# hohMiyazawa/hoh-ANS

Measured on NVIDIA B200. Metric: raw RGB MB/s, encode+decode (BASELINE.json: raw RGB MB/s encode & decode, % of HBM peak), higher is better.
Workload: dtype u8/u16 pixels, u32 freqs, u64 rANS state (integer)

## Files before the change

hoh-ans_b200/build.py:

```python
import os
import shutil
import subprocess
import sys

HERE = os.path.dirname(os.path.abspath(__file__))
CSRC = os.path.join(HERE, "csrc")
LIB = os.path.join(CSRC, "libhohgpu.so")
SOURCES = ["hoh_api.cu"]
DEPS = ["hoh_api.cu", "hoh_kernels.cuh", "hoh_format.cuh", os.path.join("..", "..", "include", "hohgpu.h")]


def nvcc_path():
    for cand in (shutil.which("nvcc"), "/usr/local/cuda/bin/nvcc"):
        if cand and os.path.exists(cand):
            return cand
    raise RuntimeError("nvcc not found")


def stale():
    if not os.path.exists(LIB):
        return True
    t = os.path.getmtime(LIB)
    return any(os.path.getmtime(os.path.join(CSRC, d)) > t for d in DEPS)


def build(force=False, verbose=False):
    if not force and not stale():
        return LIB
    cmd = [nvcc_path(), "-gencode", "arch=compute_100a,code=sm_100a", "-lineinfo", "-O3", "-std=c++17",
           "-Xcompiler", "-fPIC", "-shared", "-cudart", "static", "-o", LIB] + SOURCES
    if verbose:
        cmd.insert(1, "-Xptxas=-v")
    subprocess.check_call(cmd, cwd=CSRC)
    return LIB


if __name__ == "__main__":
    print(build(force="--force" in sys.argv, verbose="-v" in sys.argv))
```

hoh-ans_b200/csrc/hoh_api.cu:

```cuda
#include <cuda_runtime.h>

#include <algorithm>
#include <cmath>
#include <cstdio>
#include <cstdlib>
#include <cstring>
#include <map>
#include <string>
#include <vector>

#include "hoh_kernels.cuh"

using namespace hohk;

namespace {

enum Slot {
    S_FREQS = 0, S_CUM, S_HEADS, S_ENCMETA, S_DECMETA, S_RESID, S_STREAMS, S_DSTREAMS, S_DRESULTS,
    S_IO_A, S_IO_B, S_IO_C, S_IO_D, S_IO_E, S_RESULTS, S_TOP, S_BP, S_HIST, S_COST, S_SUMS, S_MASKS,
    S_WIDE_TOP, S_WIDE_BP, S_MISC, S_L_MAPS, S_L_IDX, S_L_HDR, S_L_U32, S_L_STATUS, S_L_RR, S_L_RES, S_LZ_PX, S_LZ_STATE, S_LZ_SIDE, S_LZ_COUNTS, S_LZ_SLABS, S_LZ_RES, S_LZ_BONUS, S_LZ_KEYS, S_LZ_VALS, S_LZ_FLAG, S_T_NUKE, S_T_LZ, S_T_U32, S_T_P8, S_T_P9, S_T_O8, S_T_O9, S_T_R8, S_T_R9, S_T_MORE_SHAPES, S_T_LAST = S_T_NUKE + 4 * 9 - 1, S_D_TILES, S_D_PLANES, S_D_LZSYM, S_D_IDXSYM, S_D_RESID, S_D_OUT, S_D_BACKREF, S_D_MAPS,
    S_D_STREAMS, S_D_RES_A, S_D_RES_B, S_D_TOP, S_D_BP, S_D_PSTATUS, S_L_NEED, S_L_ORDER, S_R_SLOTS, S_R_STATUS, S_COUNT
};

struct Buf {
// ... 441 lines not shown
namespace {
int predict_all_parallel(hoh_ctx* ctx, const uint16_t* d_planes, size_t n_planes, int w, int h, int depth, int x_tiles,
                         int y_tiles, const uint16_t* d_tile_maps, uint16_t* d_resid, uint64_t resid_stride) {
    const uint64_t tpr = ((uint64_t)w + kPaTx - 1) / kPaTx, tpp = tpr * (((uint64_t)h + kPaTy - 1) / kPaTy);
    if (n_planes * tpp > 0x7fffffffull) return HOH_E_UNSUPPORTED;
    k_predict_all_fused<<<(unsigned)(n_planes * tpp), 256, 0, ctx->stream>>>(
        d_planes, n_planes, w, h, depth, x_tiles, y_tiles, d_tile_maps, d_resid, resid_stride, fastdiv_make((uint32_t)tpp),
        fastdiv_make((uint32_t)tpr), fastdiv_make((uint32_t)((w + x_tiles - 1) / x_tiles)),
        fastdiv_make((uint32_t)((h + y_tiles - 1) / y_tiles)));
    LAUNCHED("k_predict_all_fused");
    return HOH_OK;
}

template <typename T>
int stage_in(hoh_ctx* ctx, Slot slot, const T* host, size_t count, T** dev) {
    TRY(scratch_t(ctx, slot, count ? count : 1, dev));
    if (count) CK(cudaMemcpyAsync(*dev, host, count * sizeof(T), cudaMemcpyHostToDevice, ctx->stream));
    return HOH_OK;
}
template <typename T>
int stage_out(hoh_ctx* ctx, T* host, const T* dev, size_t count) {
    if (count) CK(cudaMemcpyAsync(host, dev, count * sizeof(T), cudaMemcpyDeviceToHost, ctx->stream));
    CK(cudaStreamSynchronize(ctx->stream));
    return HOH_OK;
}
}

namespace {
int new_shape(hoh_ctx* ctx, uint64_t key, uint64_t& slot) {
    if (slot == key) return HOH_OK;
    if (slot != 0) {
        CK(cudaStreamSynchronize(ctx->stream));
        hoh_ctx* who[3] = {ctx, ctx->child[0], ctx->child[1]};
        for (hoh_ctx* c : who) {
            if (!c) continue;
            CK(cudaStreamSynchronize(c->stream));
            for (auto& b : c->scratch) {
                if (b.p) CK(cudaFree(b.p));
                b.p = nullptr;
                b.cap = 0;
            }
        }
    }
    slot = key;
    return HOH_OK;
}

int child_of(hoh_ctx* ctx, int k, hoh_ctx** out) {
    if (!ctx->child[k]) {
        if (hoh_ctx_create(ctx->device, nullptr, &ctx->child[k]) != HOH_OK) return HOH_E_CUDA;
        ctx->child[k]->parent = ctx;
    }
    *out = ctx->child[k];
    return HOH_OK;
}
}

extern "C" {

int hoh_ctx_create(int device, void* cuda_stream, hoh_ctx** out) {
    if (!out) return HOH_E_ARG;
    *out = nullptr;
    int count = 0;
    cudaError_t e = cudaGetDeviceCount(&count);
    if (e != cudaSuccess || count <= 0 || device < 0 || device >= count) return HOH_E_CUDA;
    if (cudaSetDevice(device) != cudaSuccess) return HOH_E_CUDA;
    hoh_ctx* ctx = new hoh_ctx();
    ctx->device = device;
    if (cudaDeviceGetAttribute(&ctx->sm_count, cudaDevAttrMultiProcessorCount, device) != cudaSuccess || ctx->sm_count <= 0)
        ctx->sm_count = 148;
    if (cuda_stream) {
        ctx->stream = reinterpret_cast<cudaStream_t>(cuda_stream);
    } else {
        if (cudaStreamCreateWithFlags(&ctx->stream, cudaStreamNonBlocking) != cudaSuccess) {
            delete ctx;
            return HOH_E_CUDA;
        }
        ctx->own_stream = true;
    }
    *out = ctx;
    return HOH_OK;
}

void hoh_ctx_destroy(hoh_ctx* ctx) {
    if (!ctx) return;
    cudaSetDevice(ctx->device);
    cudaStreamSynchronize(ctx->stream);
    for (auto& b : ctx->scratch)
        if (b.p) cudaFree(b.p);
    for (auto& kv : ctx->e_tabs) cudaFree(kv.second);
    if (ctx->flush) cudaFree(ctx->flush);
    if (ctx->d_layer_stats) cudaFree(ctx->d_layer_stats);
    for (auto& pair : ctx->ev)
        for (auto& ev : pair)
            if (ev) cudaEventDestroy(ev);
    for (auto ev : ctx->prof_events) cudaEventDestroy(ev);
    for (auto ev : ctx->prof_pool) cudaEventDestroy(ev);
    for (hoh_ctx* ch : ctx->child)
        if (ch) hoh_ctx_destroy(ch);
    if (ctx->s_h2d) cudaStreamDestroy(ctx->s_h2d);
    if (ctx->s_d2h) cudaStreamDestroy(ctx->s_d2h);
    for (int k = 0; k < kPipeDepth; k++) {
        if (ctx->ev_h2d[k]) cudaEventDestroy(ctx->ev_h2d[k]);
        if (ctx->ev_comp[k]) cudaEventDestroy(ctx->ev_comp[k]);
        if (ctx->ev_d2h[k]) cudaEventDestroy(ctx->ev_d2h[k]);
        if (ctx->ev_off[k]) cudaEventDestroy(ctx->ev_off[k]);
        if (ctx->h_off[k]) cudaFreeHost(ctx->h_off[k]);
    }
    if (ctx->ev_start) cudaEventDestroy(ctx->ev_start);
    for (int k = 0; k < 8; k++) {
        if (ctx->aux[k]) cudaStreamDestroy(ctx->aux[k]);
        if (ctx->ev_join[k]) cudaEventDestroy(ctx->ev_join[k]);
    }
    if (ctx->ev_fork) cudaEventDestroy(ctx->ev_fork);
    if (ctx->own_stream) cudaStreamDestroy(ctx->stream);
    delete ctx;
}

int hoh_release_scratch(hoh_ctx* ctx) {
    DeviceGuard guard_(ctx);
    if (!ctx) return HOH_E_ARG;
    CK(cudaStreamSynchronize(ctx->stream));
    for (auto& b : ctx->scratch) {
        if (b.p) CK(cudaFree(b.p));
        b.p = nullptr;
        b.cap = 0;
    }
    for (hoh_ctx* ch : ctx->child)
        if (ch) TRY(hoh_release_scratch(ch));
    return HOH_OK;
}

int hoh_sync(hoh_ctx* ctx) {
    DeviceGuard guard_(ctx);
    if (!ctx) return HOH_E_ARG;
    CK(cudaStreamSynchronize(ctx->stream));
    return HOH_OK;
}

const char* hoh_strerror(int status) {
    switch (status) {
        case HOH_OK: return "ok";
        case HOH_E_CUDA: return "CUDA runtime error (no device, or a call failed)";
        case HOH_E_ARG: return "bad argument";
        case HOH_E_UNSUPPORTED: return "outside the supported domain of the hot path";
        case HOH_E_CAPACITY: return "output buffer too small";
        case HOH_E_STREAM: return "a stream failed (see per-stream status)";
        default: return "unknown status";
    }
}

const char* hoh_last_cuda_error(hoh_ctx* ctx) { return ctx ? ctx->err : "no context"; }
uint64_t hoh_launch_count(hoh_ctx* ctx) { return ctx ? ctx->launches : 0; }

int hoh_debug_layer_stats(hoh_ctx* ctx, uint64_t out[3]) {
    if (!ctx || !out) return HOH_E_ARG;
    DeviceGuard guard_(ctx);
    out[0] = out[1] = out[2] = 0;
    hoh_ctx* all[5] = {ctx, ctx->child[0], ctx->child[1], ctx->child[2], ctx->child[3]};
    for (hoh_ctx* c : all) {
        if (!c || !c->d_layer_stats) continue;
        uint32_t v[4];
        CK(cudaStreamSynchronize(c->stream));
        CK(cudaMemcpy(v, c->d_layer_stats, sizeof v, cudaMemcpyDeviceToHost));
        CK(cudaMemset(c->d_layer_stats, 0, sizeof v));
        for (int k = 0; k < 3; k++) out[k] += v[k];
    }
    return HOH_OK;
}

int hoh_dev_alloc(hoh_ctx* ctx, size_t bytes, void** dptr) {
    DeviceGuard guard_(ctx);
    if (!ctx || !dptr) return HOH_E_ARG;
    CK(cudaSetDevice(ctx->device));
    CK(cudaMalloc(dptr, bytes ? bytes : 16));
    return HOH_OK;
}
int hoh_dev_free(hoh_ctx* ctx, void* dptr) {
    DeviceGuard guard_(ctx);
    if (!ctx) return HOH_E_ARG;
    CK(cudaStreamSynchronize(ctx->stream));
    CK(cudaFree(dptr));
    return HOH_OK;
}
int hoh_dev_memset(hoh_ctx* ctx, void* dptr, int value, size_t bytes) {
    DeviceGuard guard_(ctx);
    if (!ctx) return HOH_E_ARG;
    CK(cudaMemsetAsync(dptr, value, bytes, ctx->stream));
    return HOH_OK;
}
int hoh_host_alloc(hoh_ctx* ctx, size_t bytes, void** hptr) {
    DeviceGuard guard_(ctx);
    if (!ctx || !hptr) return HOH_E_ARG;
    CK(cudaHostAlloc(hptr, bytes ? bytes : 16, cudaHostAllocDefault));
    return HOH_OK;
}
int hoh_host_free(hoh_ctx* ctx, void* hptr) {
    DeviceGuard guard_(ctx);
    if (!ctx) return HOH_E_ARG;
    CK(cudaFreeHost(hptr));
    return HOH_OK;
}
int hoh_h2d(hoh_ctx* ctx, void* dst_dev, const void* src_host, size_t bytes) {
    DeviceGuard guard_(ctx);
    if (!ctx) return HOH_E_ARG;
    CK(cudaMemcpyAsync(dst_dev, src_host, bytes, cudaMemcpyHostToDevice, ctx->stream));
    return HOH_OK;
}
int hoh_d2h(hoh_ctx* ctx, void* dst_host, const void* src_dev, size_t bytes) {
    DeviceGuard guard_(ctx);
    if (!ctx) return HOH_E_ARG;
    CK(cudaMemcpyAsync(dst_host, src_dev, bytes, cudaMemcpyDeviceToHost, ctx->stream));
    return HOH_OK;
}
int hoh_timer_start(hoh_ctx* ctx, int slot) {
    DeviceGuard guard_(ctx);
    if (!ctx || slot < 0 || slot >= 16) return HOH_E_ARG;
    for (int k = 0; k < 2; k++)
        if (!ctx->ev[slot][k]) CK(cudaEventCreate(&ctx->ev[slot][k]));
    CK(cudaEventRecord(ctx->ev[slot][0], ctx->stream));
    return HOH_OK;
}
int hoh_timer_stop(hoh_ctx* ctx, int slot) {
    DeviceGuard guard_(ctx);
    if (!ctx || slot < 0 || slot >= 16 || !ctx->ev[slot][1]) return HOH_E_ARG;
    CK(cudaEventRecord(ctx->ev[slot][1], ctx->stream));
    return HOH_OK;
}
int hoh_timer_elapsed_ms(hoh_ctx* ctx, int slot, float* ms) {
    DeviceGuard guard_(ctx);
    if (!ctx || slot < 0 || slot >= 16 || !ms || !ctx->ev[slot][1]) return HOH_E_ARG;
    CK(cudaEventSynchronize(ctx->ev[slot][1]));
    CK(cudaEventElapsedTime(ms, ctx->ev[slot][0], ctx->ev[slot][1]));
    return HOH_OK;
}
int hoh_profile_begin(hoh_ctx* ctx) {
    DeviceGuard guard_(ctx);
    if (!ctx) return HOH_E_ARG;
    for (auto ev : ctx->prof_events) ctx->prof_pool.push_back(ev);
    ctx->prof_events.clear();
    ctx->prof_names.clear();
    ctx->prof_keys.clear();
    ctx->prof_ms.clear();
    ctx->prof_launches.clear();
    TRY(prof_mark(ctx, nullptr));
    ctx->profiling = true;
    return HOH_OK;
}
int hoh_profile_end(hoh_ctx* ctx) {
    DeviceGuard guard_(ctx);
    if (!ctx || !ctx->profiling) return HOH_E_ARG;
    ctx->profiling = false;
    CK(cudaStreamSynchronize(ctx->stream));
    for (size_t i = 0; i + 1 < ctx->prof_events.size(); i++) {
        float ms = 0.f;
        CK(cudaEventElapsedTime(&ms, ctx->prof_events[i], ctx->prof_events[i + 1]));
        const std::string key = ctx->prof_names[i];
        size_t k = 0;
        while (k < ctx->prof_keys.size() && ctx->prof_keys[k] != key) k++;
        if (k == ctx->prof_keys.size()) {
            ctx->prof_keys.push_back(key);
            ctx->prof_ms.push_back(0.0);
            ctx->prof_launches.push_back(0);
        }
        ctx->prof_ms[k] += ms;
        ctx->prof_launches[k]++;
    }
    return HOH_OK;
}
int hoh_profile_count(hoh_ctx* ctx) { return ctx ? (int)ctx->prof_keys.size() : 0; }
int hoh_profile_entry(hoh_ctx* ctx, int index, const char** name, double* total_ms, uint64_t* launches) {
    DeviceGuard guard_(ctx);
    if (!ctx || index < 0 || index >= (int)ctx->prof_keys.size()) return HOH_E_ARG;
    if (name) *name = ctx->prof_keys[index].c_str();
    if (total_ms) *total_ms = ctx->prof_ms[index];
    if (launches) *launches = ctx->prof_launches[index];
    return HOH_OK;
}
int hoh_flush_l2(hoh_ctx* ctx) {
    DeviceGuard guard_(ctx);
    if (!ctx) return HOH_E_ARG;
    if (!ctx->flush) {
        ctx->flush_bytes = 256ull << 20;
        CK(cudaMalloc(&ctx->flush, ctx->flush_bytes));
    }
    CK(cudaMemsetAsync(ctx->flush, 0x5a, ctx->flush_bytes, ctx->stream));
    return HOH_OK;
}

size_t hoh_enc_slab_bytes(size_t n, uint32_t prob_bits) {
    size_t payload = ((n * (size_t)prob_bits + 31) / 32) * 4 + 64;
    size_t total = payload + HOH_HEAD_CAP + 64;
    size_t stored = n * 2 + 64;
    if (stored > total) total = stored;
    return (total + 15) & ~(size_t)15;
}

int hoh_encode_entropy_batch(hoh_ctx* ctx, const hoh_enc_stream* d_streams, size_t n_streams,
                             const uint16_t* d_symbols, uint8_t* d_out, hoh_stream_result* d_results,
                             uint32_t max_range, uint32_t max_prob_bits, uint32_t max_n) {
    DeviceGuard guard_(ctx);
    if (!ctx || !d_streams || !d_out || !d_results) return HOH_E_ARG;
    if (n_streams == 0) return HOH_OK;
    if (max_range == 0 || max_range > HOH_MAX_RANGE || max_prob_bits == 0 || max_prob_bits > HOH_MAX_PROB_BITS)
        return HOH_E_UNSUPPORTED;
    (void)max_n;
// ... 1750 lines not shown
```

hoh-ans_b200/csrc/hoh_kernels.cuh:

```cuda
#pragma once
#include <cuda_runtime.h>
#include <stdint.h>

#include <cassert>
#include <type_traits>

#include "../../include/hohgpu.h"
#include "hoh_format.cuh"

namespace hohk {

constexpr int kFreqRow = 512;
constexpr int kCumRow = 520;
constexpr int kChunk = 64;
static_assert(true, "");
constexpr int kGroup = 8;
constexpr int kSymStride = 66;
constexpr uint64_t kRansL = 1ull << 31;
constexpr int kDecChunk = 32;
constexpr int kDecStride = 34;
constexpr uint32_t kSymBits = 9;
constexpr uint32_t kSymMask = (1u << kSymBits) - 1u;

struct EncMeta {
// ... 638 lines not shown
    const uint32_t s = blockIdx.x * 32u + lane;
    const bool exists = s < n_streams;
    hoh_enc_stream st;
    EncMeta m;
    if (exists) {
        st = streams[s];
        m = meta[s];
    } else {
        st.n = 0;
        st.range = 1;
        st.prob_bits = 1;
        st.sym_off = 0;
        st.out_off = 0;
        st.out_cap = 0;
        m.status = HOH_S_OK;
        m.table_u16 = want_u16;
        m.win_lo = 0;
        m.win_rows = 0;
    }
    bool live = exists && st.n > 0 && m.status == HOH_S_OK && m.table_u16 == want_u16;
    uint32_t need = live ? m.win_rows : 0u;
#pragma unroll
    for (int d = 16; d > 0; d >>= 1) need = max(need, __shfl_xor_sync(0xffffffffu, need, d));
    if (need <= rows_lo || need > rows) return;
    uint32_t low = live ? st.prob_bits : 32u;
#pragma unroll
    for (int d = 16; d > 0; d >>= 1) low = min(low, __shfl_xor_sync(0xffffffffu, low, d));
    if ((low < 14u) != LOW_BITS) return;
    if (live && (uint64_t)st.out_cap < rans_words_bound(st.n, st.prob_bits) * 4u + HOH_HEAD_CAP + 32u) {
        m.status = HOH_S_OVERFLOW;
        meta[s] = m;
        live = false;
    }
    s_off[lane] = st.sym_off;
    s_n[lane] = live ? st.n : 0u;
    if (lane == 0) {
        mbar_init(&s_bar[0], 1);
        mbar_init(&s_bar[1], 1);
        mbar_fence_init();
    }
    __syncwarp();

    for (uint32_t j = 0; j < 32; j++) {
        const uint32_t sj = blockIdx.x * 32u + j;
        const bool lj = __shfl_sync(0xffffffffu, (int)live, j) != 0;
        const uint32_t wj = __shfl_sync(0xffffffffu, m.win_rows, j);
        const uint32_t oj = __shfl_sync(0xffffffffu, m.win_lo, j);
        if (!lj) continue;
        const uint32_t* src = cumtab + (size_t)sj * kCumRow + oj;
        for (uint32_t i = lane; i < wj; i += 32) tab[i * 32u + j] = (CumT)src[i];
    }

    const PerLaneTable<CumT> T{tab, lane};
    const uint32_t bits = st.prob_bits;
    uint32_t* words = reinterpret_cast<uint32_t*>(out + st.out_off);
    const uint32_t cap_words = st.out_cap / 4u;
    uint32_t widx = cap_words;
    uint64_t x = kRansL;

    uint32_t n_max = s_n[lane];
#pragma unroll
    for (int d = 16; d > 0; d >>= 1) n_max = max(n_max, __shfl_xor_sync(0xffffffffu, n_max, d));
    const uint32_t my_n = live ? st.n : 0u;
    const uint32_t full = 1u << bits;
    const uint32_t win_lo = m.win_lo;
    const uint32_t sym_max = live ? m.win_rows - 2u : 0u;

    const int n_chunks = (int)((n_max + kChunk - 1) / kChunk);
    constexpr int kGroupsPerChunk = kChunk / kGroup;
    const uint16_t* my_sym = symbols + st.sym_off;
    uint32_t bar_parity = 0;
    uint32_t bulk_loaded = 0;
    auto load_chunk = [&](int chunk) {
        const uint32_t b = (uint32_t)chunk & 1u, first = (uint32_t)chunk * kChunk;
        const uint32_t left = my_n > first ? my_n - first : 0u;
        uint16_t* buf = stage0 + b * 32 * kBulkStride;
        if (__any_sync(0xffffffffu, left > 0u && left < (uint32_t)kChunk)) {
            stage_load_chunk<kBulkStride>(buf, symbols, s_off, s_n, (uint32_t)chunk);
            bulk_loaded &= ~(1u << b);
        } else {
            const uint32_t rows_in = __popc(__ballot_sync(0xffffffffu, left != 0u));
            fence_proxy_async();
            if (left) bulk_g2s(buf + lane * kBulkStride, my_sym + first, kChunk * 2u, &s_bar[b]);
            if (lane == 0) mbar_expect_tx(&s_bar[b], rows_in * kChunk * 2u);
            bulk_loaded |= 1u << b;
        }
    };
    auto wait_chunk = [&](int chunk) {
        const uint32_t b = (uint32_t)chunk & 1u;
        if (bulk_loaded & (1u << b)) {
            mbar_wait(&s_bar[b], (bar_parity >> b) & 1u);
            bar_parity ^= 1u << b;
            __syncwarp();
        } else {
            stage_wait();
        }
    };
    auto group_words = [&](int g) -> uint4 {
        const int chunk = g / kGroupsPerChunk, k0 = (g % kGroupsPerChunk) * kGroup;
        return *reinterpret_cast<const uint4*>(stage0 + (chunk & 1) * 32 * kBulkStride + lane * kBulkStride + k0);
    };
    auto prepare_one = [&](int g, int j, const uint4& v, uint32_t& o_start, uint32_t& o_freq, double& o_inv) {
        const uint32_t w = j < 2 ? v.x : (j < 4 ? v.y : (j < 6 ? v.z : v.w));
        const bool on = (uint32_t)g * kGroup + (uint32_t)j < my_n;
        const uint32_t raw = (j & 1) ? (w >> 16) : (w & 0xffffu);
        const uint32_t sym = on ? min(raw - win_lo, sym_max) : 0u;
        const uint32_t c0 = T.cum(sym), c1 = T.cum(sym + 1u);
        o_start = on ? c0 : 0u;
        o_freq = on ? c1 - c0 : full;
        o_inv = recip_low(o_freq);
    };
    auto prepare = [&](int g, uint32_t(&g_start)[kGroup], uint32_t(&g_freq)[kGroup], double(&g_inv)[kGroup]) {
        const uint4 v = group_words(g);
#pragma unroll
        for (int j = 0; j < kGroup; j++) prepare_one(g, j, v, g_start[j], g_freq[j], g_inv[j]);
    };
    auto run = [&](const uint32_t(&g_start)[kGroup], const uint32_t(&g_freq)[kGroup], const double(&g_inv)[kGroup]) {
#pragma unroll
        for (int j = kGroup - 1; j >= 0; j--)
            x = rans_put<LOW_BITS ? 1 : 0>(x, g_start[j], g_freq[j], g_inv[j], bits, words, widx);
    };
    if (n_chunks > 0) {
        uint32_t a_start[kGroup], a_freq[kGroup], b_start[kGroup], b_freq[kGroup];
        double a_inv[kGroup], b_inv[kGroup];
        load_chunk(n_chunks - 1);
        wait_chunk(n_chunks - 1);
        if (n_chunks > 1) load_chunk(n_chunks - 2);
        const int n_groups = n_chunks * kGroupsPerChunk;
        prepare(n_groups - 1, a_start, a_freq, a_inv);
        for (int g = n_groups - 1; g >= 1; g -= 2) {
            prepare(g - 1, b_start, b_freq, b_inv);
            run(a_start, a_freq, a_inv);
            if (g - 1 >= 1) {
                if (((g - 1) % kGroupsPerChunk) == 0) {
                    const int chunk = (g - 1) / kGroupsPerChunk;
                    wait_chunk(chunk - 1);
                    if (chunk >= 2) load_chunk(chunk - 2);
                }
                prepare(g - 2, a_start, a_freq, a_inv);
            }
            run(b_start, b_freq, b_inv);
        }
    }
    if (live) {
        widx -= 2;
        words[widx] = (uint32_t)x;
        words[widx + 1] = (uint32_t)(x >> 32);
        m.payload_start = st.out_off + (uint64_t)widx * 4u;
        m.payload_bytes = (cap_words - widx) * 4u;
        meta[s] = m;
    }
}

constexpr int kWsGroup = 8;
template <int ID>
__device__ __forceinline__ void bar_sync_named() { asm volatile("bar.sync %0, 64;" ::"n"(ID) : "memory"); }
template <int ID>
__device__ __forceinline__ void bar_arrive_named() { asm volatile("bar.arrive %0, 64;" ::"n"(ID) : "memory"); }

template <typename CumT, int DIV>
__global__ void __launch_bounds__(64) k_rans_encode_ws(const hoh_enc_stream* __restrict__ streams, uint32_t n_streams,
                                                       const uint16_t* __restrict__ symbols,
                                                       const uint32_t* __restrict__ cumtab, uint8_t* __restrict__ out,
                                                       EncMeta* __restrict__ meta, uint32_t rows_lo, uint32_t rows,
                                                       uint32_t want_u16, const uint32_t* __restrict__ order,
                                                       const uint32_t* __restrict__ n_active) {
    extern __shared__ __align__(16) uint8_t smem_raw[];
    CumT* tab = reinterpret_cast<CumT*>(smem_raw);
    uint4* hand = reinterpret_cast<uint4*>(smem_raw + (size_t)rows * 32u * sizeof(CumT));

    const uint32_t lane = lane_id();
    const bool feeder = threadIdx.x >= 32u;
    const uint32_t slot = blockIdx.x * 32u + lane;
    const uint32_t n_slots = order ? *n_active : n_streams;
    if (blockIdx.x * 32u >= n_slots) return;
    const bool exists = slot < n_slots;
    const uint32_t s = exists ? (order ? order[slot] : slot) : 0u;
    hoh_enc_stream st;
    EncMeta m;
    if (exists) {
        st = streams[s];
        m = meta[s];
    } else {
        st.n = 0;
        st.range = 1;
        st.prob_bits = 1;
        st.sym_off = 0;
        st.out_off = 0;
        st.out_cap = 0;
        m.status = HOH_S_OK;
        m.table_u16 = want_u16;
        m.win_lo = 0;
        m.win_rows = 0;
    }
    bool live = exists && st.n > 0 && m.status == HOH_S_OK && m.table_u16 == want_u16;
    uint32_t need = live ? m.win_rows : 0u;
    uint32_t low = live ? st.prob_bits : 32u;
#pragma unroll
    for (int d = 16; d > 0; d >>= 1) {
        need = max(need, __shfl_xor_sync(0xffffffffu, need, d));
        low = min(low, __shfl_xor_sync(0xffffffffu, low, d));
    }
    if (need <= rows_lo || need > rows) return;
    if ((low >= 14u ? 0 : (low >= 12u ? 2 : 1)) != DIV) return;
    if (live && (uint64_t)st.out_cap < rans_words_bound(st.n, st.prob_bits) * 4u + HOH_HEAD_CAP + 32u) {
        m.status = HOH_S_OVERFLOW;
        if (!feeder) meta[s] = m;
        live = false;
    }
    for (uint32_t j = 0; j < 32; j++) {
        const uint32_t sj = __shfl_sync(0xffffffffu, s, j);
        const bool lj = __shfl_sync(0xffffffffu, (int)live, j) != 0;
        const uint32_t wj = __shfl_sync(0xffffffffu, m.win_rows, j);
        const uint32_t oj = __shfl_sync(0xffffffffu, m.win_lo, j);
        if (!lj) continue;
        const uint32_t* src = cumtab + (size_t)sj * kCumRow + oj;
        for (uint32_t i = threadIdx.x; i < wj; i += 64) tab[i * 32u + j] = (CumT)src[i];
    }
    __syncthreads();

    const uint32_t bits = st.prob_bits;
    const uint32_t my_n = live ? st.n : 0u;
    uint32_t n_max = my_n;
#pragma unroll
    for (int d = 16; d > 0; d >>= 1) n_max = max(n_max, __shfl_xor_sync(0xffffffffu, n_max, d));
    const int n_groups = (int)((n_max + kWsGroup - 1) / kWsGroup);

    if (feeder) {
        const PerLaneTable<CumT> T{tab, lane};
        const uint32_t full = 1u << bits;
        const uint32_t win_lo = m.win_lo;
        const uint32_t sym_max = live ? m.win_rows - 2u : 0u;
        const uint16_t* my_sym = symbols + st.sym_off;
        auto load = [&](int g) -> uint4 {
            if (g >= 0 && (uint32_t)g * kWsGroup < my_n) return __ldg(reinterpret_cast<const uint4*>(my_sym + (size_t)g * kWsGroup));
            return make_uint4(0u, 0u, 0u, 0u);
        };
        uint4 set0 = load(n_groups - 1), set1 = load(n_groups - 2);
        auto feed = [&](int g, auto buf, uint4& mine) {
            constexpr int b = decltype(buf)::value;
            const uint4 cur = mine;
            uint32_t o_start[kWsGroup], o_freq[kWsGroup];
            double o_inv[kWsGroup];
#pragma unroll
            for (int j = 0; j < kWsGroup; j++) {
                const uint32_t w = j < 2 ? cur.x : (j < 4 ? cur.y : (j < 6 ? cur.z : cur.w));
                const bool on = (uint32_t)g * kWsGroup + (uint32_t)j < my_n;
                const uint32_t raw = (j & 1) ? (w >> 16) : (w & 0xffffu);
                const uint32_t sym = on ? min(raw - win_lo, sym_max) : 0u;
                const uint32_t c0 = T.cum(sym), c1 = T.cum(sym + 1u);
                o_start[j] = on ? c0 : 0u;
                o_freq[j] = on ? c1 - c0 : full;
                o_inv[j] = recip_low(o_freq[j]);
            }
            mine = load(g - 2);
            bar_sync_named<b>();
            uint4* dst = hand + (b * kWsGroup) * 32 + lane;
#pragma unroll
            for (int j = 0; j < kWsGroup; j++)
                dst[j * 32] = make_uint4(o_start[j], o_freq[j], (uint32_t)__double2loint(o_inv[j]), (uint32_t)__double2hiint(o_inv[j]));
            bar_arrive_named<2 + b>();
        };
        for (int g = n_groups - 1; g >= 0; g -= 2) {
            feed(g, std::integral_constant<int, 0>{}, set0);
            if (g >= 1) feed(g - 1, std::integral_constant<int, 1>{}, set1);
        }
        return;
    }

    uint32_t* words = reinterpret_cast<uint32_t*>(out + st.out_off);
    const uint32_t cap_words = st.out_cap / 4u;
    uint32_t widx = cap_words;
    uint64_t x = kRansL;
    bar_arrive_named<0>();
    bar_arrive_named<1>();
    auto code = [&](auto buf) {
        constexpr int b = decltype(buf)::value;
        bar_sync_named<2 + b>();
        const uint4* src = hand + (b * kWsGroup) * 32 + lane;
        uint4 h[kWsGroup];
#pragma unroll
        for (int j = 0; j < kWsGroup; j++) h[j] = src[j * 32];
        bar_arrive_named<b>();
#pragma unroll
        for (int j = kWsGroup - 1; j >= 0; j--)
            x = rans_put<DIV>(x, h[j].x, h[j].y, __hiloint2double((int)h[j].w, (int)h[j].z), bits, words, widx);
    };
    for (int it = 0; it < n_groups; it += 2) {
        code(std::integral_constant<int, 0>{});
        if (it + 1 < n_groups) code(std::integral_constant<int, 1>{});
    }
    if (live) {
        widx -= 2;
        words[widx] = (uint32_t)x;
        words[widx + 1] = (uint32_t)(x >> 32);
        m.payload_start = st.out_off + (uint64_t)widx * 4u;
        m.payload_bytes = (cap_words - widx) * 4u;
        meta[s] = m;
    }
}

__global__ void __launch_bounds__(128) k_finish_streams(const hoh_enc_stream* __restrict__ streams,
                                                        uint32_t n_streams, const uint16_t* __restrict__ symbols,
                                                        const uint8_t* __restrict__ heads,
                                                        const EncMeta* __restrict__ meta, uint8_t* __restrict__ out,
                                                        hoh_stream_result* __restrict__ results,
                                                        const uint32_t* __restrict__ order,
                                                        const uint32_t* __restrict__ n_active) {
    const uint32_t slot = blockIdx.x * 4u + (threadIdx.x >> 5), lane = lane_id();
    if (slot >= (order ? *n_active : n_streams)) return;
    const uint32_t s = order ? order[slot] : slot;
    const hoh_enc_stream st = streams[s];
    const EncMeta m = meta[s];
    const uint8_t* head = heads + (size_t)s * HOH_HEAD_CAP;
    hoh_stream_result res;
    res.status = m.status;
    res.payload_bytes = 0;
    res.stored = 0;
    res.start = st.out_off;
    res.size = 0;
    if (m.status != HOH_S_OK) {
        if (lane == 0) results[s] = res;
        return;
    }
    if (st.n == 0) {
        uint8_t* dst = out + st.out_off;
        if (lane == 0) {
            for (uint32_t k = 0; k < st.prefix_len; k++) dst[k] = st.prefix[k];
            for (uint32_t k = 0; k < m.head_len; k++) dst[st.prefix_len + k] = head[k];
            res.size = st.prefix_len + m.head_len;
            results[s] = res;
        }
        return;
    }
    {
        const uint32_t w = (m.payload_bytes - 8u) / 4u, lo = m.est & 0xffffffu, span = m.est >> 24;
        if (span != 255u && (w < lo || w > lo + span)) res.status = HOH_S_BAD_ESTIMATE;
    }
    const uint32_t vlen = hohfmt::varint_len(m.payload_bytes);
    const uint32_t coded = m.head_len + vlen + m.payload_bytes;
    if (m.stored_size < coded) {
        uint8_t* dst = out + st.out_off;
        const uint32_t maxbits = hohfmt::bit_length(st.range - 1);
        uint32_t at = st.prefix_len;
        if (lane == 0) {
            for (uint32_t k = 0; k < st.prefix_len; k++) dst[k] = st.prefix[k];
            uint32_t a = hohfmt::put_varint(dst, at, st.range - 1);
            a = hohfmt::put_varint(dst, a, st.n);
            dst[a] = 0;
        }
        at += hohfmt::varint_len(st.range - 1) + hohfmt::varint_len(st.n) + 1u;
        const uint32_t body = (uint32_t)(((uint64_t)maxbits * st.n + 7) / 8);
        const uint16_t* sym = symbols + st.sym_off;
        for (uint32_t b = lane; b < body; b += 32) {
            uint32_t byte = 0;
            for (uint32_t k = 0; k < 8; k++) {
                const uint64_t bit = (uint64_t)b * 8u + k;
                const uint64_t i = bit / maxbits;
                uint32_t v = 0;
                if (i < st.n) v = (sym[i] >> (maxbits - 1u - (uint32_t)(bit % maxbits))) & 1u;
                byte = (byte << 1) | v;
            }
            dst[at + b] = (uint8_t)byte;
        }
        res.size = st.prefix_len + m.stored_size;
        res.stored = 1;
        if (lane == 0) results[s] = res;
        return;
    }
    const uint32_t front = st.prefix_len + m.head_len + vlen;
    uint8_t* dst = out + m.payload_start - front;
    for (uint32_t k = lane; k < st.prefix_len; k += 32) dst[k] = st.prefix[k];
    for (uint32_t k = lane; k < m.head_len; k += 32) dst[st.prefix_len + k] = head[k];
    if (lane == 0) {
        hohfmt::put_varint(dst, st.prefix_len + m.head_len, m.payload_bytes);
        res.start = m.payload_start - front;
        res.size = front + m.payload_bytes;
        res.payload_bytes = m.payload_bytes;
        results[s] = res;
    }
}

__global__ void __launch_bounds__(kTableWarps * 32) k_parse_streams(
    const hoh_dec_stream* __restrict__ streams, uint32_t n_streams, const uint8_t* __restrict__ in,
    uint64_t in_bytes, uint32_t* __restrict__ cumtab, DecMeta* __restrict__ meta,
    hoh_dec_result* __restrict__ results) {
    __shared__ uint32_t s_f[kTableWarps][kFreqRow];
    __shared__ uint32_t s_cum[kTableWarps][kFreqRow + 8];
    const uint32_t w = threadIdx.x >> 5, lane = lane_id();
    const uint32_t s = blockIdx.x * kTableWarps + w;
    if (s >= n_streams) return;
    const hoh_dec_stream st = streams[s];
    const ByteView bytes{in, in_bytes};
    uint32_t* f = s_f[w];
    uint32_t* cum = s_cum[w];

    hohfmt::StreamHead h;
    uint64_t after_table = 0;
    int status = HOH_S_OK;
    uint32_t* clamps = s_cum[w];
    uint64_t field_bit = 0;
    if (lane == 0) {
        h = hohfmt::parse_head(bytes, st.in_off, st.flags);
        after_table = h.body;
        field_bit = h.body * 8u;
        if (!h.empty && h.rans) {
            if (h.range > HOH_MAX_RANGE) {
                status = HOH_S_BAD_TABLE;
            } else if (h.table_mode == 2) {
                hohfmt::BitSource<ByteView> bits{bytes, h.body, 0, 0};
                uint32_t count = (uint32_t)(((int)h.prob_bits - 1) / 4 + 2);
                if (count > 16u) count = 16u;
                clamps[0] = count;
                for (uint32_t j = 0; j < count; j++) {
                    const uint32_t lo = bits.get(h.maxbits) & 0xffffu;
                    const uint32_t hi = bits.get(h.maxbits) & 0xffffu;
                    clamps[1 + j] = lo | (hi << 16);
                }
                field_bit += 2ull * count * h.maxbits;
            } else if (h.table_mode == 3) {
                status = HOH_S_BAD_TABLE;
            }
            if ((st.flags & HOH_FIX_CARRY) && h.table_mode == 2u && status == HOH_S_OK && h.prob_bits >= 1u &&
                h.prob_bits <= HOH_MAX_PROB_BITS) {
                const uint32_t count = clamps[0];
                uint32_t v[32];
                for (uint32_t j = 0; j < count; j++) {
                    v[2u * j] = clamps[1 + j] & 0xffffu;
                    v[2u * j + 1u] = clamps[1 + j] >> 16;
                }
                hohfmt::BitSource<ByteView> bits{bytes, h.body, 0, 0};
                for (uint32_t j = 0; j < 2u * count; j++) bits.get(h.maxbits);
                const uint32_t field = bits.get(h.prob_bits);
                uint32_t rem = (2u * count * h.maxbits) & 7u;
                bool borrow = true;
                for (int j = (int)(2u * count) - 1; j >= 0 && rem && borrow; j--) {
                    const uint32_t t = min(rem, h.maxbits), mask = (1u << t) - 1u;
                    uint32_t part = v[j] & mask;
                    if (part == 0u) part = mask;
                    else {
                        part--;
                        borrow = false;
                    }
                    v[j] = (v[j] & ~mask) | part;
// ... 3696 lines not shown
    uint32_t have = 0;
    const uint32_t sbits = m.maxbits;

    const uint64_t t_glob = (uint64_t)blockIdx.x * kFusedTiles + min(tl, (uint32_t)kFusedTiles - 1u);
    const uint64_t image = t_glob / g.tiles_per_image;
    const uint32_t tile = (uint32_t)(t_glob % g.tiles_per_image);
    const uint32_t x0 = (tile % g.x_tiles) * g.tile_w, y0 = (tile / g.x_tiles) * g.tile_h;
    uint8_t* img = rgb + image * (uint64_t)g.width * g.height * 3u;
    const uint64_t row_bytes = (uint64_t)g.width * 3u;
    uint8_t* tile0 = img + ((uint64_t)y0 * g.width + x0) * 3u;
    const uint32_t half = ch == 0u ? 128u : 256u, cmask = ch == 0u ? 255u : 511u;
    const uint32_t own_shift = ch == 0u ? 8u : (ch == 1u ? 0u : 16u);
    const uint32_t g_keep = ch == 0u ? 0u : 0xffffffffu, hi_keep = ch == 0u ? 0u : 0x01010101u;
    const uint32_t my_stage_s = (uint32_t)__cvta_generic_to_shared(stage + tl * 24u + (own_shift >> 3));
    const uint2* my_out_src = reinterpret_cast<const uint2*>(stage + tl * 24u + 8u * ch);
    const uint64_t row_skip = row_bytes - (uint64_t)(tw - 8u) * 3u;
    uint8_t* p_cur = tile0;
    uint8_t* p_px = tile0 + 8u * ch;

    uint32_t L = half, TLv = half;
    uint2 ta = make_uint2(0x80808080u, 0x80808080u), tb = ta, tc = ta;
    const uint32_t groups = npx / 8u;
    uint32_t gx = 0, gy = 0;
    uint32_t v_pend = 0, gv_pend = 0;
    auto pixel_part1 = [&](uint32_t r, uint32_t t, bool row_start) {
        if (row_start) {
            L = half;
            TLv = half;
        }
        const uint32_t grad = t + L - TLv;
        const uint32_t med = max(min(t, L), min(max(t, L), grad));
        const uint32_t v = (r + med - half) & cmask;
        TLv = t;
        L = v;
        v_pend = v;
        gv_pend = __shfl_sync(0xffffffffu, v, base_lane);
    };
    auto pixel_part2 = [&](uint32_t slot) {
        asm volatile("st.shared.u8 [%0], %1;" ::"r"(my_stage_s + 3u * slot), "r"(v_pend + (gv_pend & g_keep)) : "memory");
    };
    uint32_t t01 = 0, t23 = 0, t45 = 0, t67 = 0;
    const uint32_t own_sel1 = ch == 0u ? 0x0741u : (ch == 1u ? 0x0630u : 0x0052u);
    const uint32_t own_sel2 = ch == 0u ? 0x6210u : (ch == 1u ? 0x5210u : 0x7410u);
    auto t_prepare = [&](uint2 a, uint2 b, uint2 c) {
        const uint32_t g03 = __byte_perm(__byte_perm(a.x, a.y, 0x0741), b.x, 0x6210);
        const uint32_t g47 = __byte_perm(__byte_perm(b.y, c.x, 0x0741), c.y, 0x6210);
        const uint32_t o03 = __byte_perm(__byte_perm(a.x, a.y, own_sel1), b.x, own_sel2);
        const uint32_t o47 = __byte_perm(__byte_perm(b.y, c.x, own_sel1), c.y, own_sel2);
        const uint32_t lo03 = __vsub4(o03, g03 & g_keep), lo47 = __vsub4(o47, g47 & g_keep);
        const uint32_t hi03 = __vcmpgeu4(o03, g03) & hi_keep, hi47 = __vcmpgeu4(o47, g47) & hi_keep;
        t01 = __byte_perm(lo03, hi03, 0x5140);
        t23 = __byte_perm(lo03, hi03, 0x7362);
        t45 = __byte_perm(lo47, hi47, 0x5140);
        t67 = __byte_perm(lo47, hi47, 0x7362);
    };
    auto t_of = [&](uint32_t i) -> uint32_t {
        const uint32_t pair = i < 2u ? t01 : (i < 4u ? t23 : (i < 6u ? t45 : t67));
        return (i & 1u) ? (pair >> 16) : (pair & 0xffffu);
    };
    uint32_t slot = 0, key = 0, p_lut = 0;
    auto lookup_begin = [&]() {
        slot = (uint32_t)x & mask;
        key = (slot + 1u) << kSymBits;
        if (sizeof(LutT) == 1) {
            asm volatile("ld.shared.u8 %0, [%1];" : "=r"(p_lut) : "r"(lut_s + (slot >> lut_shift) * 32u));
        } else {
            asm volatile("ld.shared.u16 %0, [%1];" : "=r"(p_lut) : "r"(lut_s + (slot >> lut_shift) * 64u));
        }
    };
    auto step = [&](auto has_stored, uint32_t i, bool row_start) {
        uint32_t em, e0, e1, e2;
        TS.at4(p_lut, em, e0, e1, e2);
        pixel_part2((i + 7u) & 7u);
        const bool down = e0 >= key;
        const bool up = e1 < key;
        uint32_t e = down ? em : (up ? e1 : e0);
        uint32_t up_ones;
        asm("set.lt.u32.u32 %0, %1, %2;" : "=r"(up_ones) : "r"(e1), "r"(key));
        uint32_t hi = down ? e0 : e1 + ((e2 - e1) & up_ones);
        const bool near = e < key && hi >= key;
        const uint64_t top = x >> bits;
        uint64_t next = (uint64_t)((hi >> kSymBits) - (e >> kSymBits)) * top + (slot - (e >> kSymBits));
        if (__builtin_expect(__any_sync(0xffffffffu, !near), 0)) {
            const ulonglong2 fixed = rans_far_step(TS, key, p_lut, e, hi, top, slot);
            next = fixed.x;
            e = (uint32_t)fixed.y;
        }
        x = next;
        const bool refill = ((uint32_t)(x >> 32) | ((uint32_t)x >> 31)) == 0u;
        x = refill ? ((x << 32) | rd.next) : x;
        rd.take_if(refill);
        uint32_t r = e & kSymMask;
        if (decltype(has_stored)::value) {
            const bool fill = stored && have < sbits;
            if (fill) {
                acc |= (uint64_t)__byte_perm(rd.next, 0u, 0x0123) << (32u - have);
                have += 32u;
            }
            rd.take_if(fill);
            if (stored) {
                r = (uint32_t)(acc >> (64u - sbits));
                acc <<= sbits;
                have -= sbits;
            }
        }
        lookup_begin();
        pixel_part1(r, t_of(i), row_start);
    };
    auto flush_group = [&]() {
        __syncwarp();
        const uint2 v = *my_out_src;
        asm volatile(
            "{\n"
            ".reg .pred p;\n"
            "setp.ne.u32 p, %3, 0;\n"
            "@p st.global.v2.u32 [%0], {%1, %2};\n"
            "}\n" ::"l"(p_px),
            "r"(v.x), "r"(v.y), "r"((uint32_t)tile_ok)
            : "memory");
        __syncwarp();
    };
    auto run = [&](auto has_stored) {
    for (uint32_t grp = 0; grp < groups; grp++) {
        rd.top_up();
        uint32_t nx = gx + 8u, ny = gy;
        const bool wrap = nx == tw;
        if (wrap) {
            nx = 0u;
            ny++;
        }
        uint8_t* p_next = p_cur + (wrap ? row_skip : 24ull);
        t_prepare(ta, tb, tc);
        step(has_stored, 0u, gx == 0u);
        flush_group();
        uint2 na = make_uint2(0x80808080u, 0x80808080u), nb = na, nc = na;
        if (ny > 0u && ny < th && tile_ok) {
            const uint2* src = reinterpret_cast<const uint2*>(p_next - row_bytes);
            na = __ldcg(src);
            nb = __ldcg(src + 1);
            nc = __ldcg(src + 2);
        }
#pragma unroll
        for (uint32_t i = 1; i < 8u; i++) step(has_stored, i, false);
        p_px = p_cur + 8u * ch;
        p_cur = p_next;
        ta = na;
        tb = nb;
        tc = nc;
        gx = nx;
        gy = ny;
    }
    };
    lookup_begin();
    if (any_stored) {
        run(StoredYes{});
    } else {
        run(StoredNo{});
    }
    pixel_part2(7u);
    flush_group();
    if (coded && x != kRansL) my_status = HOH_S_BAD_STATE;
    if (exists) status[s] = my_status;
}

__global__ void __launch_bounds__(64) k_tile_unpredict_s0_backref(const uint16_t* __restrict__ resid, TileGeom g,
                                                                  uint64_t n_tiles, const hoh_dec_result* __restrict__ res,
                                                                  const uint16_t* __restrict__ backref,
                                                                  uint16_t* __restrict__ planes,
                                                                  int32_t* __restrict__ status) {
    const uint64_t s = blockIdx.x * (uint64_t)blockDim.x + threadIdx.x;
    if (s >= n_tiles * 3u) return;
    if (status[s] != HOH_S_OK) return;
    const uint64_t t = s / 3u;
    const uint32_t ch = (uint32_t)(s % 3u);
    uint32_t x0, y0, tw, th;
    tile_rect(g, (uint32_t)(t % g.tiles_per_image), x0, y0, tw, th);
    const int c = ch == 0 ? 256 : 512, half = c >> 1;
    const uint16_t* r = resid + s * (uint64_t)g.plane_stride;
    const uint16_t* br = backref + t * (uint64_t)g.plane_stride;
    uint16_t* o = planes + s * (uint64_t)g.plane_stride;
    const uint32_t have = res[s].n;
    uint32_t k = 0;
    bool bad = false;
    for (uint32_t y = 0; y < th; y++)
        for (uint32_t x = 0; x < tw; x++) {
            const uint32_t at = y * tw + x;
            const uint32_t b = br[at];
            if (b) {
                if (b > at) {
                    bad = true;
                    o[at] = (uint16_t)half;
                } else {
                    o[at] = o[at - b];
                }
                continue;
            }
            const int L = x ? o[at - 1] : half;
            const int T = y ? o[at - tw] : half;
            const int TL = (x && y) ? o[at - tw - 1] : half;
            const int rv = k < have ? r[k] : half;
            k++;
            o[at] = (uint16_t)((rv + p_med_grad(T, L, TL) - half) & (c - 1));
        }
    if (bad || k != have) status[s] = HOH_S_BAD_LAYER;
}

__global__ void __launch_bounds__(256) k_tile_store_s0(const uint16_t* __restrict__ planes, TileGeom g,
                                                       uint8_t* __restrict__ rgb) {
    const uint64_t t = blockIdx.x;
    const uint64_t image = t / g.tiles_per_image;
    uint32_t x0, y0, tw, th;
    tile_rect(g, (uint32_t)(t % g.tiles_per_image), x0, y0, tw, th);
    uint8_t* img = rgb + image * (uint64_t)g.width * g.height * 3u;
    const uint16_t* a = planes + (t * 3u) * (uint64_t)g.plane_stride;
    const uint16_t* b = a + g.plane_stride;
    const uint16_t* c = b + g.plane_stride;
    for (uint32_t i = threadIdx.x; i < tw * th; i += blockDim.x) {
        const uint32_t x = i % tw, y = i / tw;
        uint8_t* o = img + ((uint64_t)(y0 + y) * g.width + x0 + x) * 3u;
        const uint32_t gr = a[i];
        o[1] = (uint8_t)gr;
        o[0] = (uint8_t)((b[i] + gr - 256u) & 255u);
        o[2] = (uint8_t)((c[i] + gr - 256u) & 255u);
    }
}

}
```

Before: 265,700.

## Pick encoder coder warp by hardware warpid and add warp-uniform full-group feed path

In the warp-specialized rANS encoder, the coder/feeder role is now chosen from the hardware %warpid of warp 0 rather than fixed by thread index. The intent is to place the latency-critical coder warp on a favorable SM sub-partition relative to other resident blocks. The feeder also gains a fast path, taken when all lanes have a full group, that skips per-symbol bounds masking, and it reads the cumulative table through a raw per-lane pointer. Timing probes behind a compile flag record SM, warp id and cycle counts. This adds a block-wide barrier and shared variable, and relies on %warpid, which the PTX documentation describes as volatile and not guaranteed stable.

Result: faster. 271,200 (median of 6 runs) (+2.1%).

```diff
diff --git a/hoh-ans_b200/build.py b/hoh-ans_b200/build.py
--- a/hoh-ans_b200/build.py
+++ b/hoh-ans_b200/build.py
@@ -24,15 +24,16 @@
     return any(os.path.getmtime(os.path.join(CSRC, d)) > t for d in DEPS)
 
 
-def build(force=False, verbose=False):
-    if not force and not stale():
+def build(force=False, verbose=False, out=None, defines=()):
+    if out is None and not force and not stale():
         return LIB
+    out = out or LIB
     cmd = [nvcc_path(), "-gencode", "arch=compute_100a,code=sm_100a", "-lineinfo", "-O3", "-std=c++17",
-           "-Xcompiler", "-fPIC", "-shared", "-cudart", "static", "-o", LIB] + SOURCES
+           "-Xcompiler", "-fPIC", "-shared", "-cudart", "static", "-o", out] + ["-D" + d for d in defines] + SOURCES
     if verbose:
         cmd.insert(1, "-Xptxas=-v")
     subprocess.check_call(cmd, cwd=CSRC)
-    return LIB
+    return out
 
 
 if __name__ == "__main__":
diff --git a/hoh-ans_b200/csrc/hoh_api.cu b/hoh-ans_b200/csrc/hoh_api.cu
--- a/hoh-ans_b200/csrc/hoh_api.cu
+++ b/hoh-ans_b200/csrc/hoh_api.cu
@@ -617,6 +617,24 @@
 
 const char* hoh_last_cuda_error(hoh_ctx* ctx) { return ctx ? ctx->err : "no context"; }
 uint64_t hoh_launch_count(hoh_ctx* ctx) { return ctx ? ctx->launches : 0; }
+
+#ifdef HOH_PROBE_PLACEMENT
+int hoh_probe_take(hoh_ctx* ctx, void* host, uint32_t cap, uint32_t* n) {
+    if (!ctx || !host || !n) return HOH_E_ARG;
+    DeviceGuard guard_(ctx);
+    static_assert(sizeof(ProbeRec) == 48, "hoh_probe_take's record size");
+    unsigned int count = 0;
+    if (cudaDeviceSynchronize() != cudaSuccess ||
+        cudaMemcpyFromSymbol(&count, g_probe_n, sizeof(count)) != cudaSuccess)
+        return HOH_E_CUDA;
+    const uint32_t take = min(min(count, cap), kProbeMax);
+    if (take && cudaMemcpyFromSymbol(host, g_probe, take * sizeof(ProbeRec)) != cudaSuccess) return HOH_E_CUDA;
+    const unsigned int zero = 0;
+    if (cudaMemcpyToSymbol(g_probe_n, &zero, sizeof(zero)) != cudaSuccess) return HOH_E_CUDA;
+    *n = count;
+    return HOH_OK;
+}
+#endif
 
 int hoh_debug_layer_stats(hoh_ctx* ctx, uint64_t out[3]) {
     if (!ctx || !out) return HOH_E_ARG;
diff --git a/hoh-ans_b200/csrc/hoh_kernels.cuh b/hoh-ans_b200/csrc/hoh_kernels.cuh
--- a/hoh-ans_b200/csrc/hoh_kernels.cuh
+++ b/hoh-ans_b200/csrc/hoh_kernels.cuh
@@ -814,6 +814,26 @@
     }
 }
 
+#ifdef HOH_PROBE_PLACEMENT
+struct ProbeRec {
+    uint32_t smid, warpid, role, block;
+    uint32_t warp, groups, rows, pad;
+    unsigned long long t0, t1;
+};
+constexpr uint32_t kProbeMax = 1u << 18;
+__device__ ProbeRec g_probe[kProbeMax];
+__device__ unsigned int g_probe_n;
+__device__ __forceinline__ void probe_record(uint32_t role, uint32_t groups, uint32_t rows, unsigned long long t0) {
+    const unsigned long long t1 = clock64();
+    if (lane_id() != 0) return;
+    uint32_t smid, warpid;
+    asm volatile("mov.u32 %0, %%smid;" : "=r"(smid));
+    asm volatile("mov.u32 %0, %%warpid;" : "=r"(warpid));
+    const unsigned k = atomicAdd(&g_probe_n, 1u);
+    if (k < kProbeMax) g_probe[k] = ProbeRec{smid, warpid, role, blockIdx.x, threadIdx.x >> 5, groups, rows, 0u, t0, t1};
+}
+#endif
+
 constexpr int kWsGroup = 8;
 template <int ID>
 __device__ __forceinline__ void bar_sync_named() { asm volatile("bar.sync %0, 64;" ::"n"(ID) : "memory"); }
@@ -831,8 +851,15 @@
     CumT* tab = reinterpret_cast<CumT*>(smem_raw);
     uint4* hand = reinterpret_cast<uint4*>(smem_raw + (size_t)rows * 32u * sizeof(CumT));
 
+    __shared__ uint32_t s_coder;
+    if (threadIdx.x == 0) {
+        uint32_t warpid;
+        asm volatile("mov.u32 %0, %%warpid;" : "=r"(warpid));
+        s_coder = (warpid >> 2) & 1u;
+    }
+    __syncthreads();
     const uint32_t lane = lane_id();
-    const bool feeder = threadIdx.x >= 32u;
+    const bool feeder = (threadIdx.x >> 5) != s_coder;
     const uint32_t slot = blockIdx.x * 32u + lane;
     const uint32_t n_slots = order ? *n_active : n_streams;
     if (blockIdx.x * 32u >= n_slots) return;
@@ -889,7 +916,7 @@
     const int n_groups = (int)((n_max + kWsGroup - 1) / kWsGroup);
 
     if (feeder) {
-        const PerLaneTable<CumT> T{tab, lane};
+        const CumT* my_tab = tab + lane;
         const uint32_t full = 1u << bits;
         const uint32_t win_lo = m.win_lo;
         const uint32_t sym_max = live ? m.win_rows - 2u : 0u;
@@ -899,21 +926,37 @@
             return make_uint4(0u, 0u, 0u, 0u);
         };
         uint4 set0 = load(n_groups - 1), set1 = load(n_groups - 2);
+#ifdef HOH_PROBE_PLACEMENT
+        const unsigned long long t0 = clock64();
+#endif
         auto feed = [&](int g, auto buf, uint4& mine) {
             constexpr int b = decltype(buf)::value;
             const uint4 cur = mine;
             uint32_t o_start[kWsGroup], o_freq[kWsGroup];
             double o_inv[kWsGroup];
-#pragma unroll
-            for (int j = 0; j < kWsGroup; j++) {
-                const uint32_t w = j < 2 ? cur.x : (j < 4 ? cur.y : (j < 6 ? cur.z : cur.w));
-                const bool on = (uint32_t)g * kWsGroup + (uint32_t)j < my_n;
-                const uint32_t raw = (j & 1) ? (w >> 16) : (w & 0xffffu);
-                const uint32_t sym = on ? min(raw - win_lo, sym_max) : 0u;
-                const uint32_t c0 = T.cum(sym), c1 = T.cum(sym + 1u);
-                o_start[j] = on ? c0 : 0u;
-                o_freq[j] = on ? c1 - c0 : full;
-                o_inv[j] = recip_low(o_freq[j]);
+            if (__all_sync(0xffffffffu, (uint32_t)g * kWsGroup + kWsGroup <= my_n)) {
+#pragma unroll
+                for (int j = 0; j < kWsGroup; j++) {
+                    const uint32_t w = j < 2 ? cur.x : (j < 4 ? cur.y : (j < 6 ? cur.z : cur.w));
+                    const uint32_t raw = (j & 1) ? (w >> 16) : (w & 0xffffu);
+                    const uint32_t sym = min(raw - win_lo, sym_max);
+                    const uint32_t c0 = my_tab[sym * 32u], c1 = my_tab[sym * 32u + 32u];
+                    o_start[j] = c0;
+                    o_freq[j] = c1 - c0;
+                    o_inv[j] = recip_low(o_freq[j]);
+                }
+            } else {
+#pragma unroll
+                for (int j = 0; j < kWsGroup; j++) {
+                    const uint32_t w = j < 2 ? cur.x : (j < 4 ? cur.y : (j < 6 ? cur.z : cur.w));
+                    const bool on = (uint32_t)g * kWsGroup + (uint32_t)j < my_n;
+                    const uint32_t raw = (j & 1) ? (w >> 16) : (w & 0xffffu);
+                    const uint32_t sym = on ? min(raw - win_lo, sym_max) : 0u;
+                    const uint32_t c0 = my_tab[sym * 32u], c1 = my_tab[sym * 32u + 32u];
+                    o_start[j] = on ? c0 : 0u;
+                    o_freq[j] = on ? c1 - c0 : full;
+                    o_inv[j] = recip_low(o_freq[j]);
+                }
             }
             mine = load(g - 2);
             bar_sync_named<b>();
@@ -927,6 +970,9 @@
             feed(g, std::integral_constant<int, 0>{}, set0);
             if (g >= 1) feed(g - 1, std::integral_constant<int, 1>{}, set1);
         }
+#ifdef HOH_PROBE_PLACEMENT
+        probe_record(1u, (uint32_t)n_groups, rows, t0);
+#endif
         return;
     }
 
@@ -948,10 +994,16 @@
         for (int j = kWsGroup - 1; j >= 0; j--)
             x = rans_put<DIV>(x, h[j].x, h[j].y, __hiloint2double((int)h[j].w, (int)h[j].z), bits, words, widx);
     };
+#ifdef HOH_PROBE_PLACEMENT
+    const unsigned long long t0 = clock64();
+#endif
     for (int it = 0; it < n_groups; it += 2) {
         code(std::integral_constant<int, 0>{});
         if (it + 1 < n_groups) code(std::integral_constant<int, 1>{});
     }
+#ifdef HOH_PROBE_PLACEMENT
+    probe_record(0u, (uint32_t)n_groups, rows, t0);
+#endif
     if (live) {
         widx -= 2;
         words[widx] = (uint32_t)x;
@@ -4954,11 +5006,17 @@
     }
     };
     lookup_begin();
+#ifdef HOH_PROBE_PLACEMENT
+    const unsigned long long t0 = clock64();
+#endif
     if (any_stored) {
         run(StoredYes{});
     } else {
         run(StoredNo{});
     }
+#ifdef HOH_PROBE_PLACEMENT
+    probe_record(2u, groups, rows, t0);
+#endif
     pixel_part2(7u);
     flush_group();
     if (coded && x != kRansL) my_status = HOH_S_BAD_STATE;
```
